# gdonninelli/Navier-Stokes_equations

Hardware: NVIDIA B200
Metric: time-steps/s (higher is better)
Workload: dtype f64 (fp16 operator copy inside the velocity preconditioner)

## Files before the change

### navier-stokes_equations_b200/csrc/nsb200.cu

```cuda
#include "../../include/nsb200.h"

#include <cuda_runtime.h>
#include <dlfcn.h>
#include <nccl.h>
#include <nvrtc.h>

#include <algorithm>
#include <cmath>
#include <cstdlib>
#include <cstring>
#include <map>
#include <memory>
#include <string>
#include <vector>

#include "amg.hpp"
#include "small_eig.hpp"
#include "assemble.cuh"
#include "device.cuh"
#include "linalg.cuh"
#include "structure.hpp"
#include "twolevel.cuh"
#include "velstream.cuh"

// ... 242 lines not shown
  DBuf<int> seg_ptr_f, src_f, seg_ptr_c, src_c;
  DBuf<long long> land_f, land_c;
  unsigned long long seq = 0;
  const double* last_vec = nullptr;
  int total_f_vel = 0, total_f_all = 0, total_c = 0;
  DBuf<int> send_ptr_f, send_ptr_c, list_f, list_c;
  DBuf<int2> send_dst_f, send_dst_c;
  int n_int_f = 0, n_int_c = 0;
  const double* fresh_vec = nullptr;
  unsigned long long fresh_seq = 0;
};

struct VsDev {
  const VsTile* tiles;
  const uint32_t* meta;
  const int* uniq_xoff;
  const unsigned char* vals;
  int n_tiles;
};

struct PolyLevel {
  bool coarse = false;
  int nn = 0;
  long long n = 0, n_tot = 0;
  const double* dinv = nullptr;
  const int64_t* gid = nullptr;
  double *z0 = nullptr, *z1 = nullptr, *zd = nullptr, *poly = nullptr, *pin = nullptr;
  DBuf<double> probe;
  bool probe_init = false;
  std::vector<double> wr, wi;
  double ritz_lo = 0, ritz_hi = 0, ritz_im = 0, ritz_top = 0, probe_res = 1.0;
  std::vector<std::pair<double, double>> roots;
};

struct Coarse {
  DBuf<VsTile> tiles;
  DBuf<uint32_t> meta;
  DBuf<int> uniq_xoff;
  DBuf<unsigned char> vals;
  int n_tiles = 0;
  int64_t total_nq = 0;
  DBuf<long long> nbr_ptr, vedge_ptr;
  DBuf<int> nbr_vxoff, vedge_xoff, ends_xoff, send_xoff;
  DBuf<double> cvals, dinv, rc, z0, z1, zd, poly, pin, send_buf;
  std::vector<int> h_tiles_int, h_tiles_bnd, h_tile_node_ptr;
  std::vector<int64_t> gid, h_nbr_ptr, h_nbr_gid;
  bool built = false, valid = false;
};

}

struct nsb_ctx {
  int dim = 0, device = 0;
// ... 39 lines not shown
  nsb_solver_opts opt{};
  DBuf<double> vals, dinv, ctx, cell_rhs;
  DBuf<double> forcing[2];
  bool forcing_set[2] = {false, false};
  cudaLibrary_t fsrc_lib = nullptr;
  cudaKernel_t fsrc_kernel = nullptr;
  std::string fsrc_text;
  DBuf<double> fsrc_prm, fsrc_coords;
  DBuf<int> fsrc_cells;
  DBuf<unsigned int> fsrc_flag;
  bool fsrc_geom = false;
  int64_t fsrc_compiles = 0, fsrc_evals = 0;
  DBuf<unsigned char> vs_vals;
  DBuf<VsTile> d_vs_tiles;
  DBuf<uint32_t> d_vs_meta;
  int64_t vs_total_nq = 0;
  bool vs_valid = false;
  int ctx_stride = 0;
  HostCsr h_Mp, h_Kp;
  DevCsr Mp{};
  DBuf<int> Mp_ptr, Mp_col;
  DBuf<double> Mp_val, Mp_dinv;
  double Mp_lmax = 1.0;
  std::vector<std::unique_ptr<DevLevel>> amg;
  std::vector<std::unique_ptr<HaloBuf>> halo;
  int n_tiles_int = 0, n_tiles_bnd = 0;
  std::vector<int> h_tiles_int, h_tiles_bnd, h_tile_node_ptr;
  bool fused_halo = false;
  double* pin = nullptr;
  DBuf<double> coarse_inv;
// ... 181 lines not shown
template <int DIM, typename VT> void set_vs_attr() {
  const int bytes = VsLayout<DIM, VT>::SMEM_BYTES;
  CK(cudaFuncSetAttribute(k_vel_stream<DIM, VT, 2, false>, cudaFuncAttributeMaxDynamicSharedMemorySize, bytes));
  CK(cudaFuncSetAttribute(k_vel_stream<DIM, VT, 3, false>, cudaFuncAttributeMaxDynamicSharedMemorySize, bytes));
  CK(cudaFuncSetAttribute(k_vel_stream<DIM, VT, 3, true>, cudaFuncAttributeMaxDynamicSharedMemorySize, bytes));
  CK(cudaFuncSetAttribute(k_vel_stream<DIM, VT, 4, false>, cudaFuncAttributeMaxDynamicSharedMemorySize, bytes));
  CK(cudaFuncSetAttribute(k_vel_stream<DIM, VT, 4, true>, cudaFuncAttributeMaxDynamicSharedMemorySize, bytes));
}

template <int DIM, typename VT, int MODE, bool HALO>
void launch_vel_stream(nsb_ctx* c, const VsDev& D, int ntiles, const int* list, const double* x, double* y, const double* u, double* poly,
                       PolyCoef pc, const VsHalo& hx) {
  if (ntiles <= 0) return;
  const int grid = std::min(ntiles, c->num_sms);
  k_vel_stream<DIM, VT, MODE, HALO><<<grid, VS_THREADS, VsLayout<DIM, VT>::SMEM_BYTES, c->stream>>>(
      D.tiles, ntiles, list, reinterpret_cast<const VT*>(D.vals), D.meta, D.uniq_xoff, x, y, u, poly, pc, hx);
  c->launch_check();
}
template <int MODE, bool HALO>
void vel_stream(nsb_ctx* c, const VsDev& D, int ntiles, const int* list, const double* x, double* y, const double* u, double* poly, PolyCoef pc,
                const VsHalo& hx = VsHalo{}) {
  const bool h = c->opt.precond_precision == 16;
  if (c->dim == 2) {
    if (h) launch_vel_stream<2, __half, MODE, HALO>(c, D, ntiles, list, x, y, u, poly, pc, hx);
    else launch_vel_stream<2, float, MODE, HALO>(c, D, ntiles, list, x, y, u, poly, pc, hx);
  } else {
    if (h) launch_vel_stream<3, __half, MODE, HALO>(c, D, ntiles, list, x, y, u, poly, pc, hx);
    else launch_vel_stream<3, float, MODE, HALO>(c, D, ntiles, list, x, y, u, poly, pc, hx);
  }
}
VsDev fine_dev(const nsb_ctx* c);
// ... 82 lines not shown
  double theta, delta, sigma, rho;
  Cheb(double lmax, double lmin) : theta(0.5 * (lmax + lmin)), delta(0.5 * (lmax - lmin)) {
    sigma = theta / delta;
    rho = 1.0 / sigma;
  }
  void next(double& c1, double& c2) {
    const double rho_new = 1.0 / (2.0 * sigma - rho);
    c1 = rho_new * rho;
    c2 = 2.0 * rho_new / delta;
    rho = rho_new;
  }
};


VsDev fine_dev(const nsb_ctx* c) {
  return VsDev{c->d_vs_tiles.p, c->d_vs_meta.p, c->d_suniq_xoff.p, c->vs_vals.p, c->n_stiles};
}
VsDev coarse_dev(const nsb_ctx* c) {
  return VsDev{c->cg.tiles.p, c->cg.meta.p, c->cg.uniq_xoff.p, c->cg.vals.p, c->cg.n_tiles};
}

void halo_exchange_coarse(nsb_ctx* c, double* v) {
  if (c->nranks == 1) return;
  const Structure& S = c->S;
  if (c->ph.on) {
    peer_exchange(c, v, (int)S.peer.size(), c->ph.seg_ptr_c, c->ph.src_c, c->ph.land_c, c->ph.total_c);
    return;
  }
  Coarse& G = c->cg;
  const int dim = c->dim;
  const long long tp = (long long)G.send_xoff.n;
  if (tp) { k_gather_nodes<<<nblk(tp * dim, 256), 256, 0, c->stream>>>((int)tp, dim, G.send_xoff.p, v, G.send_buf.p); c->launch_check(); }
  CKN(g_nccl.GroupStart());
  long long roff = (long long)dim * S.np_own;
// ... 542 lines not shown
  {
    TilePlan P;
    const TileLimits L{TILE_MAX_NODES, TILE_MAX_IDX, TILE_MAX_UNIQ, TILE_MAX_PUNIQ, VS_MAX_BLOCKS};
    const std::string err = build_tile_plan(S, L, P);
    if (!err.empty()) throw CudaErr{err};
    VsPlan V;
    const std::string err2 = build_vel_stream(S, P, V);
    if (!err2.empty()) throw CudaErr{err2};
    c->n_stiles = P.n_tiles();
    c->d_stile_ptr.upload(P.node_ptr, c->stream);
    c->n_tiles_int = (int)P.tiles_int.size(); c->n_tiles_bnd = (int)P.tiles_bnd.size();
    c->h_tiles_int = P.tiles_int; c->h_tiles_bnd = P.tiles_bnd; c->h_tile_node_ptr = P.node_ptr;
    c->d_suniq_ptr.upload(P.uniq_ptr, c->stream); c->d_suniq_xoff.upload(P.uniq_xoff, c->stream);
    c->d_spuniq_ptr.upload(P.puniq_ptr, c->stream); c->d_spuniq_xoff.upload(P.puniq_xoff, c->stream);
    c->d_nbr_loc.upload(P.nbr_loc, c->stream); c->d_pnbr_loc.upload(P.pnbr_loc, c->stream);
    c->d_vs_tiles.upload(V.tiles, c->stream); c->d_vs_meta.upload(V.meta, c->stream);
    c->vs_total_nq = V.total_nq;
    CK(cudaStreamSynchronize(c->stream));
    c->stiles.node_ptr = c->d_stile_ptr.p;
    c->stiles.uniq_ptr = c->d_suniq_ptr.p; c->stiles.uniq_xoff = c->d_suniq_xoff.p;
    c->stiles.puniq_ptr = c->d_spuniq_ptr.p; c->stiles.puniq_xoff = c->d_spuniq_xoff.p;
    c->stiles.nbr_loc = c->d_nbr_loc.p; c->stiles.pnbr_loc = c->d_pnbr_loc.p;
  }
  c->vs_vals.alloc(vs_vals_bytes(c));
  c->vs_valid = false;
  CK(cudaStreamSynchronize(c->stream));
  if (c->dim == 2) { set_smem_attr<2>(c->tile_smem_bytes); set_vs_attr<2, float>(); set_vs_attr<2, __half>(); }
  else { set_smem_attr<3>(c->tile_smem_bytes); set_vs_attr<3, float>(); set_vs_attr<3, __half>(); }
}

void close_peer_halo(nsb_ctx* c) {
// ... 163 lines not shown
  const Structure& Sc = CL.Sc;
  for (int P = 0; P < S.np_own; ++P)
    if (Sc.nbr_ptr[P + 1] - Sc.nbr_ptr[P] > CG_MAX_NB) throw CudaErr{"a vertex has more P1 neighbours than the coarse row kernel can accumulate"};
  TilePlan P;
  const TileLimits L{TILE_MAX_NODES, TILE_MAX_IDX, TILE_MAX_UNIQ, TILE_MAX_PUNIQ, VS_MAX_BLOCKS};
  const std::string e1 = build_tile_plan(Sc, L, P);
  if (!e1.empty()) throw CudaErr{e1};
  VsPlan V;
  const std::string e2 = build_vel_stream(Sc, P, V);
  if (!e2.empty()) throw CudaErr{e2};
  cudaStream_t st = c->stream;
  const int dim = c->dim;
  G.n_tiles = P.n_tiles();
  G.total_nq = V.total_nq;
  G.h_tiles_int = P.tiles_int; G.h_tiles_bnd = P.tiles_bnd; G.h_tile_node_ptr = P.node_ptr;
  G.tiles.upload(V.tiles, st); G.meta.upload(V.meta, st); G.uniq_xoff.upload(P.uniq_xoff, st);
  std::vector<long long> t64(Sc.nbr_ptr.begin(), Sc.nbr_ptr.end()), v64(CL.vedge_ptr.begin(), CL.vedge_ptr.end());
  G.nbr_ptr.upload(t64, st); G.vedge_ptr.upload(v64, st);
  std::vector<int> vx(Sc.nbr.size()), ex(CL.vedge.size()), en(CL.node_ends.size()), sx;
  for (size_t i = 0; i < vx.size(); ++i) vx[i] = (int)S.node_xoff(S.pid_node[Sc.nbr[i]]);
  for (size_t i = 0; i < ex.size(); ++i) ex[i] = (int)S.node_xoff(CL.vedge[i]);
  for (size_t i = 0; i < en.size(); ++i) en[i] = (int)Sc.node_xoff(CL.node_ends[i]);
  for (size_t k = 0; k < S.peer.size(); ++k)
    for (int q : S.send_pids[k]) sx.push_back((int)Sc.node_xoff(q));
  G.nbr_vxoff.upload(vx, st); G.vedge_xoff.upload(ex, st); G.ends_xoff.upload(en, st); G.send_xoff.upload(sx, st);
  G.send_buf.alloc(sx.size() * dim);
  G.gid.assign(S.pid_gid.begin(), S.pid_gid.begin() + S.np_own);
  G.h_nbr_ptr.assign(Sc.nbr_ptr.begin(), Sc.nbr_ptr.end());
  G.h_nbr_gid.resize(Sc.nbr.size());
  for (size_t i = 0; i < Sc.nbr.size(); ++i) G.h_nbr_gid[i] = S.pid_gid[Sc.nbr[i]];
  CK(cudaStreamSynchronize(st));
// ... 152 lines not shown
  double* u = level == 0 ? c->w_u.p : c->cg.z0.p;
  double* y = level == 0 ? c->w_tmp.p : c->cg.z1.p;
  double* p = level == 0 ? c->w_poly.p : c->cg.poly.p;
  level_upload(c, level, xg, x);
  if (mode >= 3) level_upload(c, level, ug, u);
  if (mode == 3) level_upload(c, level, pg, p);
  const PolyCoef pc = coef ? PolyCoef{coef[0], coef[1], coef[2], coef[3]} : PolyCoef{};
  if (mode == 2) level_apply<2>(c, lv, x, y, nullptr, nullptr, pc);
  else if (mode == 3) level_apply<3>(c, lv, x, y, u, p, pc);
  else level_apply<4>(c, lv, x, y, u, nullptr, pc);
  level_download(c, level, y, yg);
  if (mode == 3) level_download(c, level, p, pg);
}

template <typename VT>
void unpack_level(nsb_ctx* c, const VsDev& D, int64_t total_nq, size_t n_uniq, std::vector<int>& node, std::vector<int>& nbr,
                  std::vector<double>& val) {
  const int dim = c->dim, PL = dim * dim;
  std::vector<VsTile> tiles(D.n_tiles);
  std::vector<uint32_t> meta((size_t)total_nq * 4);
  std::vector<int> uniq(n_uniq);
  std::vector<VT> v((size_t)total_nq * 4 * PL);
  CK(cudaMemcpyAsync(tiles.data(), D.tiles, tiles.size() * sizeof(VsTile), cudaMemcpyDeviceToHost, c->stream));
  CK(cudaMemcpyAsync(meta.data(), D.meta, meta.size() * sizeof(uint32_t), cudaMemcpyDeviceToHost, c->stream));
  CK(cudaMemcpyAsync(uniq.data(), D.uniq_xoff, uniq.size() * sizeof(int), cudaMemcpyDeviceToHost, c->stream));
  CK(cudaMemcpyAsync(v.data(), D.vals, v.size() * sizeof(VT), cudaMemcpyDeviceToHost, c->stream));
  CK(cudaStreamSynchronize(c->stream));
  for (const VsTile& T : tiles) {
    const uint32_t* m = meta.data() + (size_t)T.nq_off * 4;
    const VT* tv = v.data() + (size_t)T.nq_off * 4 * PL;
    for (int q = 0; q < T.nquad; ++q) {
      const uint32_t* mq = m + 4 * q;
      if (mq[2] == 0xffffu) continue;
      const int cnt = (int)(mq[3] >> 16);
      for (int e = 0; e < cnt; ++e) {
        const int loc = (int)(((e < 2 ? mq[0] : mq[1]) >> (16 * (e & 1))) & 0xffffu);
        node.push_back(T.n0 + (int)mq[2]);
        nbr.push_back(uniq[T.u0 + loc] / dim);
        for (int rc = 0; rc < PL; ++rc) val.push_back((double)(float)tv[((size_t)rc * T.NQ + q) * 4 + e]);
      }
    }
  }
}

size_t forcing_len(const nsb_ctx* c) { return (size_t)c->S.nc * (c->dim == 2 ? Fe<2>::NQ : Fe<3>::NQ) * c->dim; }

void forcing_alloc(nsb_ctx* c) {
  if (c->forcing[0].p) return;
  for (auto& b : c->forcing) { b.alloc(forcing_len(c)); b.zero(c->stream); }
}

void forcing_commit(nsb_ctx* c, int which, bool nonzero, bool written) {
  if (!nonzero && c->forcing_set[1 - which] && (written || c->forcing_set[which])) c->forcing[which].zero(c->stream);
// ... 776 lines not shown
  CK(cudaSetDevice(c->device));
  const Structure& S = c->S;
  const int prec = c->opt.precond_precision, PL = c->dim * c->dim;
  const int nn = level == 0 ? S.nn_own : S.np_own;
  if (precision) *precision = prec;
  if (tiles) *tiles = level == 0 ? c->n_stiles : c->cg.n_tiles;
  if (n_rows) *n_rows = nn;
  if (row_gid) for (int A = 0; A < nn; ++A) row_gid[A] = level == 0 ? S.node_gid[A] : S.pid_gid[A];
  std::vector<int> node, nbr;
  std::vector<double> v;
  if (prec != 64) {
    if (level == 0 && !c->vs_valid) return fail(c, "the packed velocity operator does not match the assembled system");
    if (level == 1 && !c->cg.valid) return fail(c, "the coarse operator has not been assembled (linearised systems with velocity_cycle = 2 only)");
    const VsDev D = level == 0 ? fine_dev(c) : coarse_dev(c);
    const int64_t nq = level == 0 ? c->vs_total_nq : c->cg.total_nq;
    const size_t nuq = level == 0 ? c->d_suniq_xoff.n : c->cg.uniq_xoff.n;
    if (prec == 16) unpack_level<__half>(c, D, nq, nuq, node, nbr, v);
    else unpack_level<float>(c, D, nq, nuq, node, nbr, v);
  }
  if (n_blocks) *n_blocks = (int64_t)node.size();
  std::vector<int64_t> rp(nn + 1, 0);
  for (int a : node) ++rp[a + 1];
  for (int A = 0; A < nn; ++A) rp[A + 1] += rp[A];
  if (rowptr) std::copy(rp.begin(), rp.end(), rowptr);
  std::vector<int64_t> cur(rp.begin(), rp.end() - 1);
  for (size_t i = 0; i < node.size(); ++i) {
    const int64_t k = cur[node[i]]++;
    if (col_gid) col_gid[k] = level == 0 ? S.node_gid[nbr[i]] : S.pid_gid[nbr[i]];
    if (vals) std::copy(v.begin() + i * PL, v.begin() + (i + 1) * PL, vals + k * PL);
  }
  return 0;
  NSB_CATCH(c)
}
// ... 175 lines not shown
                       const uint32_t* cell_dofs, int64_t n_u, int64_t n_p, const int32_t* cell_part, int rank, int nranks,
                       int64_t* out5) {
  Structure S;
  const std::string e = build_structure(dim, n_vertices, coords, n_cells, cell_vertices, cell_dofs, n_u, n_p,
                                        nranks > 1 ? cell_part : nullptr, rank, nranks, S);
  if (!e.empty()) { std::fprintf(stderr, "nsb_test_tile_plan: %s\n", e.c_str()); return -1; }
  TilePlan P;
  const TileLimits L{TILE_MAX_NODES, TILE_MAX_IDX, TILE_MAX_UNIQ, TILE_MAX_PUNIQ, VS_MAX_BLOCKS};
  const std::string e2 = build_tile_plan(S, L, P);
  if (!e2.empty()) { std::fprintf(stderr, "nsb_test_tile_plan: %s\n", e2.c_str()); return -1; }
  VsPlan V;
  const std::string e3 = build_vel_stream(S, P, V);
  if (!e3.empty()) { std::fprintf(stderr, "nsb_test_tile_plan: %s\n", e3.c_str()); return -1; }
  out5[0] = P.n_tiles(); out5[1] = (int64_t)P.tiles_int.size(); out5[2] = (int64_t)P.tiles_bnd.size();
  out5[3] = 4 * V.total_nq; out5[4] = verify_tile_plan(S, L, P) + verify_vel_stream(S, P, V);
  return 0;
}

int nsb_test_coarse_level(int dim, int64_t n_vertices, const double* coords, int64_t n_cells, const uint32_t* cell_vertices,
                          const uint32_t* cell_dofs, int64_t n_u, int64_t n_p, const int32_t* cell_part, int rank, int nranks,
                          int64_t* sizes4, int64_t* node_gid, int64_t* ends_gid, int64_t* vedge_pairs, int64_t* vertex_gid,
                          int64_t* cnbr_ptr, int64_t* cnbr_gid) {
  Structure S;
  const std::string e = build_structure(dim, n_vertices, coords, n_cells, cell_vertices, cell_dofs, n_u, n_p,
                                        nranks > 1 ? cell_part : nullptr, rank, nranks, S);
  if (!e.empty()) { std::fprintf(stderr, "nsb_test_coarse_level: %s\n", e.c_str()); return -1; }
  CoarseLevel C;
  const std::string e2 = build_coarse(S, C);
  if (!e2.empty()) { std::fprintf(stderr, "nsb_test_coarse_level: %s\n", e2.c_str()); return -1; }
  sizes4[0] = S.nn_own; sizes4[1] = (int64_t)C.vedge.size(); sizes4[2] = S.np_own; sizes4[3] = (int64_t)C.Sc.nbr.size();
// ... 21 lines not shown
  if (poly_degree) {
    int d = 0;
    for (auto& r : c->lvF.roots) d += (r.second != 0.0) ? 2 : 1;
    *poly_degree = d;
  }
  if (poly_probe_residual) *poly_probe_residual = c->lvF.probe_res;
  if (amg_levels) *amg_levels = (int)c->amg.size();
  return 0;
}

int nsb_velocity_operator_info(nsb_handle c, int* precision, int64_t* value_bytes, int64_t* index_bytes, int64_t* tiles,
                               int64_t* blocks) {
  if (!c || !c->have_mesh) return fail(c, "no mesh uploaded");
  if (precision) *precision = c->opt.precond_precision;
  if (value_bytes) *value_bytes = (int64_t)vs_vals_bytes(c);
  if (index_bytes) *index_bytes = 16 * c->vs_total_nq + 64 * (int64_t)c->n_stiles + 4 * (int64_t)c->d_suniq_xoff.n;
  if (tiles) *tiles = c->n_stiles;
  if (blocks) *blocks = (int64_t)c->S.nbr.size();
  return 0;
}

int nsb_comm_info(nsb_handle c, int* nranks, int* halo_mode, int64_t* halo_doubles_per_exchange) {
  if (!c) return -1;
  if (nranks) *nranks = c->nranks;
  if (halo_mode) *halo_mode = c->nranks == 1 ? 0 : !c->ph.on ? 1 : c->fused_halo ? 3 : 2;
  if (halo_doubles_per_exchange) {
    int64_t t = 0;
    for (size_t k = 0; k < c->S.peer.size(); ++k) t += (int64_t)c->S.send_nodes[k].size() * c->dim;
    *halo_doubles_per_exchange = t;
  }
  return 0;
// ... 48 lines not shown
```

### navier-stokes_equations_b200/csrc/structure.cpp

```cpp
#include "structure.hpp"

#include <algorithm>
#include <cstring>
#include <climits>
#include <cmath>
#include <numeric>

namespace nsb {

namespace {
struct Layout {
  int dim, NV, NN, DPC;
  int udof(int a, int c) const { return a < NV ? a * (dim + 1) + c : NV * (dim + 1) + (a - NV) * dim + c; }
  int pdof(int v) const { return v * (dim + 1) + dim; }
};
}

std::string build_structure(int dim, int64_t n_vertices, const double* coords, int64_t n_cells,
                            const uint32_t* cell_vertices, const uint32_t* cell_dofs, int64_t n_u,
                            int64_t n_p, const int32_t* cell_part, int rank, int nranks, Structure& S) {
  if (dim != 2 && dim != 3) return "dim must be 2 or 3";
  Layout L{dim, dim + 1, (dim == 2) ? 6 : 10, 0};
  L.DPC = dim * L.NN + L.NV;
  const int NV = L.NV, NN = L.NN, DPC = L.DPC;
// ... 389 lines not shown
    for (size_t i = 0; i < U.size(); ++i) { posn[U[i]] = (int)i; P.uniq_xoff.push_back((int)S.node_xoff(U[i])); }
    for (size_t i = 0; i < PU.size(); ++i) { posp[PU[i]] = (int)i; P.puniq_xoff.push_back((int)S.pid_xoff(PU[i])); }
    for (int B = start; B < A; ++B) {
      for (int64_t k = S.nbr_ptr[B]; k < S.nbr_ptr[B + 1]; ++k) P.nbr_loc[k] = (unsigned short)posn[S.nbr[k]];
      for (int64_t k = S.pnbr_ptr[B]; k < S.pnbr_ptr[B + 1]; ++k) P.pnbr_loc[k] = (unsigned short)posp[S.pnbr[k]];
    }
    bool reads_ghost = false;
    for (int n : U) reads_ghost |= (n >= S.nn_own);
    (reads_ghost ? P.tiles_bnd : P.tiles_int).push_back(tile);
    P.node_ptr.push_back(A); P.uniq_ptr.push_back((int)P.uniq_xoff.size()); P.puniq_ptr.push_back((int)P.puniq_xoff.size());
    ++tile;
  }
  return "";
}

std::string build_vel_stream(const Structure& S, const TilePlan& P, VsPlan& V) {
  V = VsPlan();
  const int nt = P.n_tiles();
  V.tiles.resize(nt);
  auto quads = [&](int A) { return (int)((S.nbr_ptr[A + 1] - S.nbr_ptr[A] + 3) / 4); };
  int64_t off = 0;
  std::vector<int> qstart;
  for (int t = 0; t < nt; ++t) {
    VsTile& T = V.tiles[t];
    std::memset(&T, 0, sizeof(T));
    T.n0 = P.node_ptr[t]; T.nn = P.node_ptr[t + 1] - T.n0;
    qstart.assign(T.nn + 1, 0);
    for (int a = 0; a < T.nn; ++a) qstart[a + 1] = qstart[a] + quads(T.n0 + a);
    if (qstart[T.nn] > VS_MAX_QUADS) return "an SpMV tile holds more velocity blocks than the streamed operator can stage";
    T.nquad = qstart[T.nn];
    T.NQ = (T.nquad + 31) / 32 * 32;
    if ((off + T.NQ) * 4 >= (int64_t)INT32_MAX) return "too many velocity blocks for 32-bit tile offsets";
    T.nq_off = (int)off;
    T.u0 = P.uniq_ptr[t]; T.nuq = P.uniq_ptr[t + 1] - T.u0;
    int a = 0;
    for (int w = 0; w <= VS_CONSUMERS; ++w) {
      const int target = (int)((int64_t)T.nquad * w / VS_CONSUMERS);
      while (a < T.nn && qstart[a] < target) ++a;
      T.split[w] = (unsigned short)qstart[a];
    }
    T.split[VS_CONSUMERS] = (unsigned short)T.nquad;
    off += T.NQ;
  }
  V.total_nq = off;
  V.meta.assign((size_t)off * 4, 0u);
#pragma omp parallel for schedule(static)
  for (int t = 0; t < nt; ++t) {
    const VsTile& T = V.tiles[t];
    uint32_t* m = V.meta.data() + (size_t)T.nq_off * 4;
    int q = 0;
    for (int a = 0; a < T.nn; ++a) {
      const int64_t k0 = S.nbr_ptr[T.n0 + a], k1 = S.nbr_ptr[T.n0 + a + 1];
      for (int64_t k = k0; k < k1; k += 4, ++q) {
        uint32_t loc[4];
        const int cnt = (int)std::min<int64_t>(4, k1 - k);
        for (int e = 0; e < 4; ++e) loc[e] = P.nbr_loc[k + (e < cnt ? e : 0)];
        m[4 * q + 0] = loc[0] | (loc[1] << 16);
        m[4 * q + 1] = loc[2] | (loc[3] << 16);
        m[4 * q + 2] = (uint32_t)a;
        m[4 * q + 3] = (uint32_t)(k - k0) | ((uint32_t)cnt << 16);
      }
    }
    for (; q < T.NQ; ++q) { m[4 * q + 0] = 0; m[4 * q + 1] = 0; m[4 * q + 2] = 0xffffu; m[4 * q + 3] = 0; }
  }
  return "";
}

int64_t verify_vel_stream(const Structure& S, const TilePlan& P, const VsPlan& V) {
  int64_t bad = 0;
  const int nt = P.n_tiles();
  if ((int)V.tiles.size() != nt) return 1;
  int64_t off = 0;
  int next_node = 0;
  for (int t = 0; t < nt; ++t) {
    const VsTile& T = V.tiles[t];
    if (T.n0 != next_node || T.nn <= 0 || T.nn > 64) ++bad;
    next_node = T.n0 + T.nn;
    if (T.nq_off != off || T.NQ % 32 || T.NQ < T.nquad || T.NQ > VS_MAX_QUADS) ++bad;
    if (T.u0 != P.uniq_ptr[t] || T.nuq != P.uniq_ptr[t + 1] - P.uniq_ptr[t]) ++bad;
    const uint32_t* m = V.meta.data() + (size_t)off * 4;
    int q = 0;
    std::vector<int> qstart(1, 0);
    for (int a = 0; a < T.nn; ++a) {
      const int64_t k0 = S.nbr_ptr[T.n0 + a], k1 = S.nbr_ptr[T.n0 + a + 1];
      for (int64_t k = k0; k < k1; k += 4, ++q) {
        const int cnt = (int)(m[4 * q + 3] >> 16), first = (int)(m[4 * q + 3] & 0xffffu);
        if ((int)m[4 * q + 2] != a || first != (int)(k - k0) || cnt != (int)std::min<int64_t>(4, k1 - k)) ++bad;
        for (int e = 0; e < 4; ++e) {
          const int loc = (int)((m[4 * q + e / 2] >> (16 * (e & 1))) & 0xffffu);
          if (loc >= T.nuq) { ++bad; continue; }
          if (e < cnt && P.uniq_xoff[T.u0 + loc] != (int)S.node_xoff(S.nbr[k + e])) ++bad;
        }
      }
      qstart.push_back(q);
    }
    if (q != T.nquad) ++bad;
    for (; q < T.NQ; ++q) if (m[4 * q + 2] != 0xffffu) ++bad;
    if (T.split[0] != 0 || T.split[VS_CONSUMERS] != T.nquad) ++bad;
    for (int w = 0; w < VS_CONSUMERS; ++w) {
      if (T.split[w] > T.split[w + 1]) ++bad;
      if (!std::binary_search(qstart.begin(), qstart.end(), (int)T.split[w])) ++bad;
    }
    off += T.NQ;
  }
  if (next_node != S.nn_own || off != V.total_nq) ++bad;
  return bad;
}

std::string build_coarse(const Structure& S, CoarseLevel& C) {
  C = CoarseLevel();
  static const int lines2[3][2] = {{0, 1}, {1, 2}, {2, 0}};
  static const int lines3[6][2] = {{0, 1}, {1, 2}, {2, 0}, {0, 3}, {1, 3}, {2, 3}};
  const int dim = S.dim, NV = S.NV, NN = S.NN, NL = NN - NV;
  Structure& Sc = C.Sc;
  Sc.dim = dim; Sc.NV = NV; Sc.NN = NN; Sc.DPC = S.DPC;
  Sc.rank = S.rank; Sc.nranks = S.nranks;
  Sc.nn_own = S.np_own; Sc.nn_ghost = S.np_ghost; Sc.np_own = 0; Sc.np_ghost = 0; Sc.nc = 0;
  Sc.node_gid = S.pid_gid;
  Sc.nbr_ptr.assign(S.np_own + 1, 0);
  for (int P = 0; P < S.np_own; ++P) {
    const int A = S.pid_node[P];
// ... 81 lines not shown
```

### navier-stokes_equations_b200/csrc/structure.hpp

```cpp
#pragma once
#include <cstdint>
#include <string>
#include <vector>

namespace nsb {

struct Structure {
  int dim = 0, NV = 0, NN = 0, DPC = 0;
  int rank = 0, nranks = 1;
  int64_t n_u_glob = 0, n_p_glob = 0, n_cells_glob = 0;
  int nn_own = 0, nn_ghost = 0, np_own = 0, np_ghost = 0, nc = 0;
  std::vector<int64_t> node_gid;
  std::vector<int64_t> pid_gid;
  std::vector<int> cell_gid;
  std::vector<int> cell_nodes;
  std::vector<int> cell_pids;
  std::vector<int> node_pid;
  std::vector<int> pid_node;
  std::vector<int64_t> nbr_ptr;
  std::vector<int> nbr;
  std::vector<int64_t> pnbr_ptr;
  std::vector<int> pnbr;
  std::vector<int> selfrank;
  std::vector<int> pselfrank;
// ... 36 lines not shown
struct TilePlan {
  std::vector<int> node_ptr;
  std::vector<int> uniq_ptr, uniq_xoff;
  std::vector<int> puniq_ptr, puniq_xoff;
  std::vector<unsigned short> nbr_loc;
  std::vector<unsigned short> pnbr_loc;
  std::vector<int> tiles_int, tiles_bnd;
  int n_tiles() const { return (int)node_ptr.size() - 1; }
};
std::string build_tile_plan(const Structure& S, const TileLimits& L, TilePlan& P);
int64_t verify_tile_plan(const Structure& S, const TileLimits& L, const TilePlan& P);

constexpr int VS_CONSUMERS = 8;
constexpr int VS_MAX_BLOCKS = 2048;
constexpr int VS_MAX_QUADS = VS_MAX_BLOCKS / 4;
struct alignas(16) VsTile {
  int n0, nn;
  int nquad, NQ;
  int nq_off;
  int u0, nuq;
  int pad0;
  unsigned short split[VS_CONSUMERS + 1];
  unsigned short pad1[32 - 16 - (VS_CONSUMERS + 1)];
};
static_assert(sizeof(VsTile) == 64, "VsTile is one 64-byte TMA bulk copy");
struct VsPlan {
  std::vector<VsTile> tiles;
  std::vector<uint32_t> meta;
  int64_t total_nq = 0;
};
std::string build_vel_stream(const Structure& S, const TilePlan& P, VsPlan& V);
int64_t verify_vel_stream(const Structure& S, const TilePlan& P, const VsPlan& V);

struct CoarseLevel {
  Structure Sc;
  std::vector<int64_t> vedge_ptr;
  std::vector<int> vedge;
  std::vector<int> node_ends;
};
std::string build_coarse(const Structure& S, CoarseLevel& C);

void export_pattern(const Structure& S, std::vector<int64_t>& rowptr, std::vector<uint32_t>& col);

void export_row_gids(const Structure& S, std::vector<int64_t>& gid);

}
```

### navier-stokes_equations_b200/csrc/velstream.cuh

```cuda
#pragma once
#include <cuda_fp16.h>

#include "device.cuh"
#include "linalg.cuh"
#include "structure.hpp"

namespace nsb {

constexpr int VS_GROUPS = 2;
constexpr int VS_THREADS = (VS_GROUPS * VS_CONSUMERS + 1) * 32;
constexpr int VS_MAX_UNIQ = TILE_MAX_UNIQ;

template <int DIM, typename VT> struct VsLayout {
  static constexpr int PL = DIM * DIM;
  static constexpr int VAL_BYTES = PL * VS_MAX_BLOCKS * (int)sizeof(VT);
  static constexpr int META_BYTES = VS_MAX_QUADS * 16;
  static constexpr int XS_BYTES = VS_MAX_UNIQ * DIM * 8;
  static constexpr int YS_BYTES = TILE_MAX_NODES * DIM * 8;
  static constexpr int HDR_BYTES = 64;
  static constexpr int OFF_VAL = 0;
  static constexpr int OFF_META = OFF_VAL + VAL_BYTES;
  static constexpr int OFF_XS = OFF_META + META_BYTES;
  static constexpr int OFF_YS = OFF_XS + XS_BYTES;
  static constexpr int OFF_HDR = OFF_YS + YS_BYTES;
  static constexpr int STAGE_BYTES = ((OFF_HDR + HDR_BYTES + 127) / 128) * 128;
  static constexpr int STAGES = (227 * 1024 - 256) / STAGE_BYTES >= 3 ? 3 : 2;
  static constexpr int SMEM_BYTES = STAGES * STAGE_BYTES + 256;
};

__device__ __forceinline__ uint32_t smem_u32(const void* p) { return (uint32_t)__cvta_generic_to_shared(p); }
__device__ __forceinline__ void mbar_init(uint64_t* bar, uint32_t count) {
  asm volatile("mbarrier.init.shared::cta.b64 [%0], %1;" ::"r"(smem_u32(bar)), "r"(count) : "memory");
}
__device__ __forceinline__ void mbar_expect_tx(uint64_t* bar, uint32_t bytes) {
  asm volatile("mbarrier.arrive.expect_tx.shared::cta.b64 _, [%0], %1;" ::"r"(smem_u32(bar)), "r"(bytes) : "memory");
}
__device__ __forceinline__ void mbar_arrive(uint64_t* bar) {
  asm volatile("mbarrier.arrive.shared::cta.b64 _, [%0];" ::"r"(smem_u32(bar)) : "memory");
}
__device__ __forceinline__ void mbar_wait(uint64_t* bar, uint32_t parity) {
  asm volatile(
      "{\n\t.reg .pred p;\n\t"
      "WAIT_%=:\n\t"
// ... 35 lines not shown
  unsigned long long wait_seq;
  int ghost_start;
  const int* send_ptr;
  const int2* send_dst;
  double* const* peer_arena;
  long long y_off;
  unsigned long long* const* peer_flags;
  int my_rank;
  unsigned long long push_seq;
  unsigned int* counter;
};

template <int DIM, typename VT, int MODE, bool HALO>
__global__ void __launch_bounds__(VS_THREADS, 1)
k_vel_stream(const VsTile* __restrict__ tiles, int n_tiles, const int* __restrict__ tile_list, const VT* __restrict__ vals,
             const uint32_t* __restrict__ meta, const int* __restrict__ uniq_xoff, const double* __restrict__ x,
             double* __restrict__ y, const double* __restrict__ u, double* __restrict__ poly, PolyCoef pc, VsHalo hx) {
  using L = VsLayout<DIM, VT>;
  constexpr int PL = L::PL;
  constexpr int S = L::STAGES;
  extern __shared__ __align__(128) unsigned char vs_smem[];
  uint64_t* full = reinterpret_cast<uint64_t*>(vs_smem + S * L::STAGE_BYTES);
  uint64_t* empty = full + S;
  const int warp = threadIdx.x >> 5, lane = threadIdx.x & 31;
  if (threadIdx.x == 0) {
    for (int s = 0; s < S; ++s) {
      mbar_init(full + s, 1 + 32);
      mbar_init(empty + s, VS_CONSUMERS);
    }
    asm volatile("fence.mbarrier_init.release.cluster;" ::: "memory");
  }
// ... 10 lines not shown
      bool ghosts = false;
      if (HALO) {
        ghosts = t >= hx.n_int;
        if (ghosts && !waited) {
          if (hx.wait_seq && lane < hx.npeers) {
            const volatile unsigned long long* f = hx.flags + hx.peer_rank[lane];
            while (*f < hx.wait_seq) { }
          }
          __threadfence_system();
          __syncwarp();
          waited = true;
        }
        t = __ldg(tile_list + t);
      }
      const VsTile* hd = tiles + t;
      const int NQ = __ldg(&hd->NQ), nq_off = __ldg(&hd->nq_off), u0 = __ldg(&hd->u0), nuq = __ldg(&hd->nuq);
      unsigned char* st = vs_smem + s * L::STAGE_BYTES;
      if (lane == 0) {
        const uint32_t vb = (uint32_t)(PL * 4 * NQ * (int)sizeof(VT)), mb = (uint32_t)(NQ * 16);
        mbar_expect_tx(full + s, vb + mb + (uint32_t)L::HDR_BYTES);
        tma_bulk_g2s(st + L::OFF_HDR, hd, L::HDR_BYTES, full + s);
        tma_bulk_g2s(st + L::OFF_VAL, vals + (long long)PL * 4 * nq_off, vb, full + s);
        tma_bulk_g2s(st + L::OFF_META, meta + (long long)4 * nq_off, mb, full + s);
      }
      double* xs = reinterpret_cast<double*>(st + L::OFF_XS);
      constexpr int PER_LANE = VS_MAX_UNIQ / 32;
      int xo[PER_LANE];
#pragma unroll
      for (int q = 0; q < PER_LANE; ++q) {
        const int i = lane + 32 * q;
        xo[q] = i < nuq ? __ldg(uniq_xoff + u0 + i) : -1;
      }
      if (HALO && ghosts) {
#pragma unroll
        for (int q0 = 0; q0 < PER_LANE; q0 += 4) {
          double gv[4][DIM];
#pragma unroll
          for (int q = q0; q < q0 + 4; ++q)
            if (xo[q] >= hx.ghost_start) {
#pragma unroll
              for (int c = 0; c < DIM; ++c) gv[q - q0][c] = __ldcg(x + xo[q] + c);
            }
#pragma unroll
          for (int q = q0; q < q0 + 4; ++q) {
            const int i = lane + 32 * q;
            if (xo[q] >= hx.ghost_start) {
// ... 210 lines not shown
```

Measured before the change: 0.4708.

## Assign bank-aware shared-memory x slots per tile to cut bank conflicts

Adds a host-side pass that places each tile's unique neighbour x values into shared-memory slots chosen to spread each warp's gathers across banks, and rewrites the meta indices and per-tile slot-to-x offset table to match. The kernel now gathers x into slots through the new table instead of the unique-neighbour list. The goal is fewer shared-memory wavefronts in the streamed velocity SpMV. The cost is more setup work, padding slots that can enlarge the staged x region and per-tile gather count, and a bank-model test hook.

```diff
diff --git a/navier-stokes_equations_b200/csrc/nsb200.cu b/navier-stokes_equations_b200/csrc/nsb200.cu
--- a/navier-stokes_equations_b200/csrc/nsb200.cu
+++ b/navier-stokes_equations_b200/csrc/nsb200.cu
@@ -280,7 +280,7 @@
 struct VsDev {
   const VsTile* tiles;
   const uint32_t* meta;
-  const int* uniq_xoff;
+  const int* slot_xoff;
   const unsigned char* vals;
   int n_tiles;
 };
@@ -302,7 +302,7 @@
 struct Coarse {
   DBuf<VsTile> tiles;
   DBuf<uint32_t> meta;
-  DBuf<int> uniq_xoff;
+  DBuf<int> slot_xoff;
   DBuf<unsigned char> vals;
   int n_tiles = 0;
   int64_t total_nq = 0;
@@ -372,6 +372,7 @@
   DBuf<unsigned char> vs_vals;
   DBuf<VsTile> d_vs_tiles;
   DBuf<uint32_t> d_vs_meta;
+  DBuf<int> d_vs_slot_xoff;
   int64_t vs_total_nq = 0;
   bool vs_valid = false;
   int ctx_stride = 0;
@@ -583,7 +584,7 @@
   if (ntiles <= 0) return;
   const int grid = std::min(ntiles, c->num_sms);
   k_vel_stream<DIM, VT, MODE, HALO><<<grid, VS_THREADS, VsLayout<DIM, VT>::SMEM_BYTES, c->stream>>>(
-      D.tiles, ntiles, list, reinterpret_cast<const VT*>(D.vals), D.meta, D.uniq_xoff, x, y, u, poly, pc, hx);
+      D.tiles, ntiles, list, reinterpret_cast<const VT*>(D.vals), D.meta, D.slot_xoff, x, y, u, poly, pc, hx);
   c->launch_check();
 }
 template <int MODE, bool HALO>
@@ -696,10 +697,10 @@
 
 
 VsDev fine_dev(const nsb_ctx* c) {
-  return VsDev{c->d_vs_tiles.p, c->d_vs_meta.p, c->d_suniq_xoff.p, c->vs_vals.p, c->n_stiles};
+  return VsDev{c->d_vs_tiles.p, c->d_vs_meta.p, c->d_vs_slot_xoff.p, c->vs_vals.p, c->n_stiles};
 }
 VsDev coarse_dev(const nsb_ctx* c) {
-  return VsDev{c->cg.tiles.p, c->cg.meta.p, c->cg.uniq_xoff.p, c->cg.vals.p, c->cg.n_tiles};
+  return VsDev{c->cg.tiles.p, c->cg.meta.p, c->cg.slot_xoff.p, c->cg.vals.p, c->cg.n_tiles};
 }
 
 void halo_exchange_coarse(nsb_ctx* c, double* v) {
@@ -1272,7 +1273,7 @@
     c->d_suniq_ptr.upload(P.uniq_ptr, c->stream); c->d_suniq_xoff.upload(P.uniq_xoff, c->stream);
     c->d_spuniq_ptr.upload(P.puniq_ptr, c->stream); c->d_spuniq_xoff.upload(P.puniq_xoff, c->stream);
     c->d_nbr_loc.upload(P.nbr_loc, c->stream); c->d_pnbr_loc.upload(P.pnbr_loc, c->stream);
-    c->d_vs_tiles.upload(V.tiles, c->stream); c->d_vs_meta.upload(V.meta, c->stream);
+    c->d_vs_tiles.upload(V.tiles, c->stream); c->d_vs_meta.upload(V.meta, c->stream); c->d_vs_slot_xoff.upload(V.slot_xoff, c->stream);
     c->vs_total_nq = V.total_nq;
     CK(cudaStreamSynchronize(c->stream));
     c->stiles.node_ptr = c->d_stile_ptr.p;
@@ -1466,7 +1467,7 @@
   G.n_tiles = P.n_tiles();
   G.total_nq = V.total_nq;
   G.h_tiles_int = P.tiles_int; G.h_tiles_bnd = P.tiles_bnd; G.h_tile_node_ptr = P.node_ptr;
-  G.tiles.upload(V.tiles, st); G.meta.upload(V.meta, st); G.uniq_xoff.upload(P.uniq_xoff, st);
+  G.tiles.upload(V.tiles, st); G.meta.upload(V.meta, st); G.slot_xoff.upload(V.slot_xoff, st);
   std::vector<long long> t64(Sc.nbr_ptr.begin(), Sc.nbr_ptr.end()), v64(CL.vedge_ptr.begin(), CL.vedge_ptr.end());
   G.nbr_ptr.upload(t64, st); G.vedge_ptr.upload(v64, st);
   std::vector<int> vx(Sc.nbr.size()), ex(CL.vedge.size()), en(CL.node_ends.size()), sx;
@@ -1649,16 +1650,16 @@
 }
 
 template <typename VT>
-void unpack_level(nsb_ctx* c, const VsDev& D, int64_t total_nq, size_t n_uniq, std::vector<int>& node, std::vector<int>& nbr,
+void unpack_level(nsb_ctx* c, const VsDev& D, int64_t total_nq, size_t n_slots, std::vector<int>& node, std::vector<int>& nbr,
                   std::vector<double>& val) {
   const int dim = c->dim, PL = dim * dim;
   std::vector<VsTile> tiles(D.n_tiles);
   std::vector<uint32_t> meta((size_t)total_nq * 4);
-  std::vector<int> uniq(n_uniq);
+  std::vector<int> slots(n_slots);
   std::vector<VT> v((size_t)total_nq * 4 * PL);
   CK(cudaMemcpyAsync(tiles.data(), D.tiles, tiles.size() * sizeof(VsTile), cudaMemcpyDeviceToHost, c->stream));
   CK(cudaMemcpyAsync(meta.data(), D.meta, meta.size() * sizeof(uint32_t), cudaMemcpyDeviceToHost, c->stream));
-  CK(cudaMemcpyAsync(uniq.data(), D.uniq_xoff, uniq.size() * sizeof(int), cudaMemcpyDeviceToHost, c->stream));
+  CK(cudaMemcpyAsync(slots.data(), D.slot_xoff, slots.size() * sizeof(int), cudaMemcpyDeviceToHost, c->stream));
   CK(cudaMemcpyAsync(v.data(), D.vals, v.size() * sizeof(VT), cudaMemcpyDeviceToHost, c->stream));
   CK(cudaStreamSynchronize(c->stream));
   for (const VsTile& T : tiles) {
@@ -1671,7 +1672,7 @@
       for (int e = 0; e < cnt; ++e) {
         const int loc = (int)(((e < 2 ? mq[0] : mq[1]) >> (16 * (e & 1))) & 0xffffu);
         node.push_back(T.n0 + (int)mq[2]);
-        nbr.push_back(uniq[T.u0 + loc] / dim);
+        nbr.push_back(slots[T.s0 + loc] / dim);
         for (int rc = 0; rc < PL; ++rc) val.push_back((double)(float)tv[((size_t)rc * T.NQ + q) * 4 + e]);
       }
     }
@@ -2478,9 +2479,9 @@
     if (level == 1 && !c->cg.valid) return fail(c, "the coarse operator has not been assembled (linearised systems with velocity_cycle = 2 only)");
     const VsDev D = level == 0 ? fine_dev(c) : coarse_dev(c);
     const int64_t nq = level == 0 ? c->vs_total_nq : c->cg.total_nq;
-    const size_t nuq = level == 0 ? c->d_suniq_xoff.n : c->cg.uniq_xoff.n;
-    if (prec == 16) unpack_level<__half>(c, D, nq, nuq, node, nbr, v);
-    else unpack_level<float>(c, D, nq, nuq, node, nbr, v);
+    const size_t ns = level == 0 ? c->d_vs_slot_xoff.n : c->cg.slot_xoff.n;
+    if (prec == 16) unpack_level<__half>(c, D, nq, ns, node, nbr, v);
+    else unpack_level<float>(c, D, nq, ns, node, nbr, v);
   }
   if (n_blocks) *n_blocks = (int64_t)node.size();
   std::vector<int64_t> rp(nn + 1, 0);
@@ -2686,6 +2687,33 @@
   if (!e3.empty()) { std::fprintf(stderr, "nsb_test_tile_plan: %s\n", e3.c_str()); return -1; }
   out5[0] = P.n_tiles(); out5[1] = (int64_t)P.tiles_int.size(); out5[2] = (int64_t)P.tiles_bnd.size();
   out5[3] = 4 * V.total_nq; out5[4] = verify_tile_plan(S, L, P) + verify_vel_stream(S, P, V);
+  return 0;
+}
+
+int nsb_test_vs_banks(int dim, int64_t n_vertices, const double* coords, int64_t n_cells, const uint32_t* cell_vertices,
+                      const uint32_t* cell_dofs, int64_t n_u, int64_t n_p, const int32_t* cell_part, int rank, int nranks,
+                      int level, int bank_slots, int64_t* out37) {
+  Structure S;
+  const std::string e = build_structure(dim, n_vertices, coords, n_cells, cell_vertices, cell_dofs, n_u, n_p,
+                                        nranks > 1 ? cell_part : nullptr, rank, nranks, S);
+  if (!e.empty()) { std::fprintf(stderr, "nsb_test_vs_banks: %s\n", e.c_str()); return -1; }
+  CoarseLevel CL;
+  if (level == 1) {
+    const std::string e1 = build_coarse(S, CL);
+    if (!e1.empty()) { std::fprintf(stderr, "nsb_test_vs_banks: %s\n", e1.c_str()); return -1; }
+  }
+  const Structure& SL = level == 1 ? CL.Sc : S;
+  TilePlan P;
+  const TileLimits L{TILE_MAX_NODES, TILE_MAX_IDX, TILE_MAX_UNIQ, TILE_MAX_PUNIQ, VS_MAX_BLOCKS};
+  const std::string e2 = build_tile_plan(SL, L, P);
+  if (!e2.empty()) { std::fprintf(stderr, "nsb_test_vs_banks: %s\n", e2.c_str()); return -1; }
+  VsPlan V;
+  const std::string e3 = build_vel_stream(SL, P, V, bank_slots != 0);
+  if (!e3.empty()) { std::fprintf(stderr, "nsb_test_vs_banks: %s\n", e3.c_str()); return -1; }
+  const VsBankCount B = vs_bank_model(SL, V);
+  out37[0] = B.loads; out37[1] = B.wavefronts; out37[2] = (int64_t)V.slot_xoff.size();
+  out37[3] = verify_tile_plan(SL, L, P) + verify_vel_stream(SL, P, V);
+  std::copy(B.hist, B.hist + 33, out37 + 4);
   return 0;
 }
 
@@ -2737,7 +2765,7 @@
   if (!c || !c->have_mesh) return fail(c, "no mesh uploaded");
   if (precision) *precision = c->opt.precond_precision;
   if (value_bytes) *value_bytes = (int64_t)vs_vals_bytes(c);
-  if (index_bytes) *index_bytes = 16 * c->vs_total_nq + 64 * (int64_t)c->n_stiles + 4 * (int64_t)c->d_suniq_xoff.n;
+  if (index_bytes) *index_bytes = 16 * c->vs_total_nq + 64 * (int64_t)c->n_stiles + 4 * (int64_t)c->d_vs_slot_xoff.n;
   if (tiles) *tiles = c->n_stiles;
   if (blocks) *blocks = (int64_t)c->S.nbr.size();
   return 0;
diff --git a/navier-stokes_equations_b200/csrc/structure.cpp b/navier-stokes_equations_b200/csrc/structure.cpp
--- a/navier-stokes_equations_b200/csrc/structure.cpp
+++ b/navier-stokes_equations_b200/csrc/structure.cpp
@@ -427,7 +427,73 @@
   return "";
 }
 
-std::string build_vel_stream(const Structure& S, const TilePlan& P, VsPlan& V) {
+static int assign_bank_slots(int dim, const VsTile& T, const uint32_t* m, int nuq, std::vector<int>& slot) {
+  const int K = vs_bank_classes(dim), cap = VS_MAX_SLOTS / K, PL = vs_pass_lanes(dim);
+  auto pos = [&](int j, int e) { return (int)((m[4 * j + e / 2] >> (16 * (e & 1))) & 0xffffu); };
+  std::vector<int> gptr(1, 0), gnode, stamp(nuq, -1);
+  for (int w = 0; w < VS_CONSUMERS; ++w)
+    for (int base = T.split[w]; base < T.split[w + 1]; base += 32)
+      for (int lo = base; lo < std::min(base + 32, (int)T.split[w + 1]); lo += PL) {
+        const int hi = std::min({lo + PL, base + 32, (int)T.split[w + 1]});
+        for (int e = 0; e < 4; ++e) {
+          const int g = (int)gptr.size() - 1;
+          for (int j = lo; j < hi; ++j) {
+            const int u = pos(j, e);
+            if (stamp[u] != g) { stamp[u] = g; gnode.push_back(u); }
+          }
+          gptr.push_back((int)gnode.size());
+        }
+      }
+  const int ng = (int)gptr.size() - 1;
+  std::vector<int> nptr(nuq + 1, 0), ngrp(gnode.size());
+  for (int u : gnode) ++nptr[u + 1];
+  for (int u = 0; u < nuq; ++u) nptr[u + 1] += nptr[u];
+  {
+    std::vector<int> fill(nptr.begin(), nptr.end() - 1);
+    for (int g = 0; g < ng; ++g)
+      for (int i = gptr[g]; i < gptr[g + 1]; ++i) ngrp[fill[gnode[i]]++] = g;
+  }
+  std::vector<int> order(nuq), cnt((size_t)ng * K, 0), mx(ng, 0), occ(K, 0), cls(nuq, -1);
+  std::iota(order.begin(), order.end(), 0);
+  std::stable_sort(order.begin(), order.end(), [&](int a, int b) { return nptr[a + 1] - nptr[a] > nptr[b + 1] - nptr[b]; });
+  auto best = [&](int u) {
+    int bk = -1;
+    int64_t bc = INT64_MAX;
+    for (int k = 0; k < K; ++k) {
+      if (occ[k] >= cap) continue;
+      int64_t hit = 0, load = 0;
+      for (int i = nptr[u]; i < nptr[u + 1]; ++i) {
+        const int g = ngrp[i], c = cnt[(size_t)g * K + k];
+        hit += c >= std::max(mx[g], 1);
+        load += c;
+      }
+      const int64_t cost = (hit << 40) + (load << 20) + occ[k];
+      if (cost < bc) { bc = cost; bk = k; }
+    }
+    return bk;
+  };
+  auto move = [&](int u, int k, int d) {
+    occ[k] += d;
+    for (int i = nptr[u]; i < nptr[u + 1]; ++i) {
+      const int g = ngrp[i];
+      int* cg = cnt.data() + (size_t)g * K;
+      cg[k] += d;
+      mx[g] = d > 0 ? std::max(mx[g], cg[k]) : *std::max_element(cg, cg + K);
+    }
+  };
+  for (int u : order) { cls[u] = best(u); move(u, cls[u], 1); }
+  for (int pass = 0; pass < 2; ++pass)
+    for (int u : order) { move(u, cls[u], -1); cls[u] = best(u); move(u, cls[u], 1); }
+  std::vector<int> fill(K, 0);
+  int nslot = 0;
+  for (int u = 0; u < nuq; ++u) {
+    slot[u] = cls[u] + K * fill[cls[u]]++;
+    nslot = std::max(nslot, slot[u] + 1);
+  }
+  return nslot;
+}
+
+std::string build_vel_stream(const Structure& S, const TilePlan& P, VsPlan& V, bool bank_slots) {
   V = VsPlan();
   const int nt = P.n_tiles();
   V.tiles.resize(nt);
@@ -441,11 +507,11 @@
     qstart.assign(T.nn + 1, 0);
     for (int a = 0; a < T.nn; ++a) qstart[a + 1] = qstart[a] + quads(T.n0 + a);
     if (qstart[T.nn] > VS_MAX_QUADS) return "an SpMV tile holds more velocity blocks than the streamed operator can stage";
+    if (P.uniq_ptr[t + 1] - P.uniq_ptr[t] > VS_MAX_SLOTS) return "an SpMV tile has more unique neighbours than the streamed operator has x slots";
     T.nquad = qstart[T.nn];
     T.NQ = (T.nquad + 31) / 32 * 32;
     if ((off + T.NQ) * 4 >= (int64_t)INT32_MAX) return "too many velocity blocks for 32-bit tile offsets";
     T.nq_off = (int)off;
-    T.u0 = P.uniq_ptr[t]; T.nuq = P.uniq_ptr[t + 1] - T.u0;
     int a = 0;
     for (int w = 0; w <= VS_CONSUMERS; ++w) {
       const int target = (int)((int64_t)T.nquad * w / VS_CONSUMERS);
@@ -457,7 +523,8 @@
   }
   V.total_nq = off;
   V.meta.assign((size_t)off * 4, 0u);
-#pragma omp parallel for schedule(static)
+  std::vector<std::vector<int>> tile_slots(nt);
+#pragma omp parallel for schedule(dynamic, 64)
   for (int t = 0; t < nt; ++t) {
     const VsTile& T = V.tiles[t];
     uint32_t* m = V.meta.data() + (size_t)T.nq_off * 4;
@@ -475,6 +542,27 @@
       }
     }
     for (; q < T.NQ; ++q) { m[4 * q + 0] = 0; m[4 * q + 1] = 0; m[4 * q + 2] = 0xffffu; m[4 * q + 3] = 0; }
+    const int u0 = P.uniq_ptr[t], nuq = P.uniq_ptr[t + 1] - u0;
+    std::vector<int> slot(nuq);
+    std::iota(slot.begin(), slot.end(), 0);
+    const int nslot = bank_slots ? assign_bank_slots(S.dim, T, m, nuq, slot) : nuq;
+    for (int j = 0; j < T.nquad; ++j)
+      for (int w = 0; w < 2; ++w) {
+        const uint32_t v = m[4 * j + w];
+        m[4 * j + w] = (uint32_t)slot[v & 0xffffu] | ((uint32_t)slot[v >> 16] << 16);
+      }
+    std::vector<int>& xo = tile_slots[t];
+    xo.assign(nslot, -1);
+    for (int u = 0; u < nuq; ++u) xo[slot[u]] = P.uniq_xoff[u0 + u];
+  }
+  int64_t soff = 0;
+  for (int t = 0; t < nt; ++t) soff += (int64_t)tile_slots[t].size();
+  if (soff >= (int64_t)INT32_MAX) return "too many x slots for 32-bit tile offsets";
+  V.slot_xoff.reserve((size_t)soff);
+  for (int t = 0; t < nt; ++t) {
+    V.tiles[t].s0 = (int)V.slot_xoff.size();
+    V.tiles[t].nslot = (int)tile_slots[t].size();
+    V.slot_xoff.insert(V.slot_xoff.end(), tile_slots[t].begin(), tile_slots[t].end());
   }
   return "";
 }
@@ -483,14 +571,19 @@
   int64_t bad = 0;
   const int nt = P.n_tiles();
   if ((int)V.tiles.size() != nt) return 1;
-  int64_t off = 0;
+  int64_t off = 0, soff = 0;
   int next_node = 0;
+  std::vector<int> uq;
   for (int t = 0; t < nt; ++t) {
     const VsTile& T = V.tiles[t];
     if (T.n0 != next_node || T.nn <= 0 || T.nn > 64) ++bad;
     next_node = T.n0 + T.nn;
     if (T.nq_off != off || T.NQ % 32 || T.NQ < T.nquad || T.NQ > VS_MAX_QUADS) ++bad;
-    if (T.u0 != P.uniq_ptr[t] || T.nuq != P.uniq_ptr[t + 1] - P.uniq_ptr[t]) ++bad;
+    if (T.s0 != soff || T.nslot < 0 || T.nslot > VS_MAX_SLOTS || soff + T.nslot > (int64_t)V.slot_xoff.size()) return bad + 1;
+    uq.clear();
+    for (int i = 0; i < T.nslot; ++i) if (V.slot_xoff[T.s0 + i] >= 0) uq.push_back(V.slot_xoff[T.s0 + i]);
+    std::sort(uq.begin(), uq.end());
+    if (!std::equal(uq.begin(), uq.end(), P.uniq_xoff.begin() + P.uniq_ptr[t], P.uniq_xoff.begin() + P.uniq_ptr[t + 1])) ++bad;
     const uint32_t* m = V.meta.data() + (size_t)off * 4;
     int q = 0;
     std::vector<int> qstart(1, 0);
@@ -501,8 +594,8 @@
         if ((int)m[4 * q + 2] != a || first != (int)(k - k0) || cnt != (int)std::min<int64_t>(4, k1 - k)) ++bad;
         for (int e = 0; e < 4; ++e) {
           const int loc = (int)((m[4 * q + e / 2] >> (16 * (e & 1))) & 0xffffu);
-          if (loc >= T.nuq) { ++bad; continue; }
-          if (e < cnt && P.uniq_xoff[T.u0 + loc] != (int)S.node_xoff(S.nbr[k + e])) ++bad;
+          if (loc >= T.nslot || V.slot_xoff[T.s0 + loc] < 0) { ++bad; continue; }
+          if (e < cnt && V.slot_xoff[T.s0 + loc] != (int)S.node_xoff(S.nbr[k + e])) ++bad;
         }
       }
       qstart.push_back(q);
@@ -515,9 +608,54 @@
       if (!std::binary_search(qstart.begin(), qstart.end(), (int)T.split[w])) ++bad;
     }
     off += T.NQ;
-  }
-  if (next_node != S.nn_own || off != V.total_nq) ++bad;
+    soff += T.nslot;
+  }
+  if (next_node != S.nn_own || off != V.total_nq || soff != (int64_t)V.slot_xoff.size()) ++bad;
   return bad;
+}
+
+VsBankCount vs_bank_model(const Structure& S, const VsPlan& V) {
+  const int dim = S.dim, PL = vs_pass_lanes(dim);
+  const int W = 16 / PL, NU = 16 / W, NC = dim / W;
+  VsBankCount R;
+#pragma omp parallel
+  {
+    VsBankCount L;
+#pragma omp for schedule(dynamic, 64)
+    for (int t = 0; t < (int)V.tiles.size(); ++t) {
+      const VsTile& T = V.tiles[t];
+      const uint32_t* m = V.meta.data() + (size_t)T.nq_off * 4;
+      for (int w = 0; w < VS_CONSUMERS; ++w)
+        for (int base = T.split[w]; base < T.split[w + 1]; base += 32)
+          for (int e = 0; e < 4; ++e)
+            for (int c = 0; c < NC; ++c) {
+              int wf = 0;
+              for (int lo = base; lo < std::min(base + 32, (int)T.split[w + 1]); lo += PL) {
+                const int hi = std::min({lo + PL, base + 32, (int)T.split[w + 1]});
+                int word[16], n = 0, per[16] = {};
+                for (int j = lo; j < hi; ++j) {
+                  const int slot = (int)((m[4 * j + e / 2] >> (16 * (e & 1))) & 0xffffu);
+                  word[n++] = (slot * dim + c * W) / W;
+                }
+                std::sort(word, word + n);
+                const int nd = (int)(std::unique(word, word + n) - word);
+                int most = 0;
+                for (int i = 0; i < nd; ++i) most = std::max(most, ++per[word[i] % NU]);
+                wf += most;
+              }
+              ++L.loads;
+              L.wavefronts += wf;
+              ++L.hist[std::min(wf, 32)];
+            }
+    }
+#pragma omp critical
+    {
+      R.loads += L.loads;
+      R.wavefronts += L.wavefronts;
+      for (int i = 0; i <= 32; ++i) R.hist[i] += L.hist[i];
+    }
+  }
+  return R;
 }
 
 std::string build_coarse(const Structure& S, CoarseLevel& C) {
diff --git a/navier-stokes_equations_b200/csrc/structure.hpp b/navier-stokes_equations_b200/csrc/structure.hpp
--- a/navier-stokes_equations_b200/csrc/structure.hpp
+++ b/navier-stokes_equations_b200/csrc/structure.hpp
@@ -74,11 +74,14 @@
 constexpr int VS_CONSUMERS = 8;
 constexpr int VS_MAX_BLOCKS = 2048;
 constexpr int VS_MAX_QUADS = VS_MAX_BLOCKS / 4;
+constexpr int VS_MAX_SLOTS = 1024;
+constexpr int vs_bank_classes(int dim) { return dim == 2 ? 8 : 16; }
+constexpr int vs_pass_lanes(int dim) { return dim == 2 ? 8 : 16; }
 struct alignas(16) VsTile {
   int n0, nn;
   int nquad, NQ;
   int nq_off;
-  int u0, nuq;
+  int s0, nslot;
   int pad0;
   unsigned short split[VS_CONSUMERS + 1];
   unsigned short pad1[32 - 16 - (VS_CONSUMERS + 1)];
@@ -87,10 +90,16 @@
 struct VsPlan {
   std::vector<VsTile> tiles;
   std::vector<uint32_t> meta;
+  std::vector<int> slot_xoff;
   int64_t total_nq = 0;
 };
-std::string build_vel_stream(const Structure& S, const TilePlan& P, VsPlan& V);
+std::string build_vel_stream(const Structure& S, const TilePlan& P, VsPlan& V, bool bank_slots = true);
 int64_t verify_vel_stream(const Structure& S, const TilePlan& P, const VsPlan& V);
+struct VsBankCount {
+  int64_t loads = 0, wavefronts = 0;
+  int64_t hist[33] = {};
+};
+VsBankCount vs_bank_model(const Structure& S, const VsPlan& V);
 
 struct CoarseLevel {
   Structure Sc;
diff --git a/navier-stokes_equations_b200/csrc/velstream.cuh b/navier-stokes_equations_b200/csrc/velstream.cuh
--- a/navier-stokes_equations_b200/csrc/velstream.cuh
+++ b/navier-stokes_equations_b200/csrc/velstream.cuh
@@ -9,13 +9,12 @@
 
 constexpr int VS_GROUPS = 2;
 constexpr int VS_THREADS = (VS_GROUPS * VS_CONSUMERS + 1) * 32;
-constexpr int VS_MAX_UNIQ = TILE_MAX_UNIQ;
 
 template <int DIM, typename VT> struct VsLayout {
   static constexpr int PL = DIM * DIM;
   static constexpr int VAL_BYTES = PL * VS_MAX_BLOCKS * (int)sizeof(VT);
   static constexpr int META_BYTES = VS_MAX_QUADS * 16;
-  static constexpr int XS_BYTES = VS_MAX_UNIQ * DIM * 8;
+  static constexpr int XS_BYTES = VS_MAX_SLOTS * DIM * 8;
   static constexpr int YS_BYTES = TILE_MAX_NODES * DIM * 8;
   static constexpr int HDR_BYTES = 64;
   static constexpr int OFF_VAL = 0;
@@ -26,7 +25,9 @@
   static constexpr int STAGE_BYTES = ((OFF_HDR + HDR_BYTES + 127) / 128) * 128;
   static constexpr int STAGES = (227 * 1024 - 256) / STAGE_BYTES >= 3 ? 3 : 2;
   static constexpr int SMEM_BYTES = STAGES * STAGE_BYTES + 256;
+  static_assert(STAGES == (DIM == 3 && sizeof(VT) == 4 ? 2 : 3), "pipeline depth: 2 stages for 3-D fp32, 3 otherwise");
 };
+static_assert(TILE_MAX_UNIQ <= VS_MAX_SLOTS, "every unique neighbour of a tile needs an x slot");
 
 __device__ __forceinline__ uint32_t smem_u32(const void* p) { return (uint32_t)__cvta_generic_to_shared(p); }
 __device__ __forceinline__ void mbar_init(uint64_t* bar, uint32_t count) {
@@ -92,7 +93,7 @@
 template <int DIM, typename VT, int MODE, bool HALO>
 __global__ void __launch_bounds__(VS_THREADS, 1)
 k_vel_stream(const VsTile* __restrict__ tiles, int n_tiles, const int* __restrict__ tile_list, const VT* __restrict__ vals,
-             const uint32_t* __restrict__ meta, const int* __restrict__ uniq_xoff, const double* __restrict__ x,
+             const uint32_t* __restrict__ meta, const int* __restrict__ slot_xoff, const double* __restrict__ x,
              double* __restrict__ y, const double* __restrict__ u, double* __restrict__ poly, PolyCoef pc, VsHalo hx) {
   using L = VsLayout<DIM, VT>;
   constexpr int PL = L::PL;
@@ -133,7 +134,7 @@
         t = __ldg(tile_list + t);
       }
       const VsTile* hd = tiles + t;
-      const int NQ = __ldg(&hd->NQ), nq_off = __ldg(&hd->nq_off), u0 = __ldg(&hd->u0), nuq = __ldg(&hd->nuq);
+      const int NQ = __ldg(&hd->NQ), nq_off = __ldg(&hd->nq_off), s0 = __ldg(&hd->s0), nslot = __ldg(&hd->nslot);
       unsigned char* st = vs_smem + s * L::STAGE_BYTES;
       if (lane == 0) {
         const uint32_t vb = (uint32_t)(PL * 4 * NQ * (int)sizeof(VT)), mb = (uint32_t)(NQ * 16);
@@ -143,12 +144,12 @@
         tma_bulk_g2s(st + L::OFF_META, meta + (long long)4 * nq_off, mb, full + s);
       }
       double* xs = reinterpret_cast<double*>(st + L::OFF_XS);
-      constexpr int PER_LANE = VS_MAX_UNIQ / 32;
+      constexpr int PER_LANE = VS_MAX_SLOTS / 32;
       int xo[PER_LANE];
 #pragma unroll
       for (int q = 0; q < PER_LANE; ++q) {
         const int i = lane + 32 * q;
-        xo[q] = i < nuq ? __ldg(uniq_xoff + u0 + i) : -1;
+        xo[q] = i < nslot ? __ldg(slot_xoff + s0 + i) : -1;
       }
       if (HALO && ghosts) {
 #pragma unroll
```

Result: slower. 0.4639, median of 6 (-1.5%).
